# uthree/tinyvc

Measured on AMD Instinct MI355X. Metric: audio-samples/sec (16 kHz) end-to-end VC, higher is better.
Workload: dtype f32 (fp32 in / out / accumulate; channel contractions as two-term fp16 splits on v_mfma_f32_32x32x16_f16: 22-bit significands, three part-products per fp32 product)

## Files before the change

### tinyvc_amd/csrc/api.hip

```cpp
#include <atomic>
#include <cmath>
#include <mutex>

#include <cstdlib>

#include "knn_blob.h"
#include "tvc_common.h"

using namespace tvc;

static std::mutex g_blob_mu;
static std::map<const void*, int64_t> g_blobs;
constexpr size_t kMaxBlobRecords = 4096;
static void blob_record(const void* p, int64_t N) {
    std::lock_guard<std::mutex> lk(g_blob_mu);
    if (g_blobs.size() >= kMaxBlobRecords && !g_blobs.count(p)) g_blobs.clear();
    g_blobs[p] = N;
}
static void blob_forget(const void* p) {
    std::lock_guard<std::mutex> lk(g_blob_mu);
    g_blobs.erase(p);
}
static int blob_check(tvc_ctx* ctx, hipStream_t s, const void* p, int64_t N, const char* what) {
    {
// ... 168 lines not shown
    float* emax = ws.get<float>((size_t)(2 + nslots) * NB);
    float* spec_bound = emax + NB;
    float* enc_slots = spec_bound + NB;
    float* srcmax = c.alpha ? enc_slots + 3 * NB : nullptr;
    float* abound = c.alpha ? ws.get<float>((size_t)NB) : nullptr;
    const int M = ix.M > 0 ? ix.M : 1;
    float* rowmax = ix.per_row ? ws.get<float>((size_t)NB) : nullptr;
    const bool auto_pitch = c.target_f0 != nullptr;
    float* rshift = ix.per_row && c.shifts && !auto_pitch ? ws.get<float>((size_t)NB) : nullptr;
    std::vector<KnnSegIn> segs;
    if (ix.per_row) {
        for (int m = 0; m < M; ++m)
            for (int i = 0; i < NB; ++i) {
                const int r = ctx->rag ? ctx->rag->row[i] : i;
                const int c0 = ctx->rag ? ctx->rag->pre[i] : i * T, nc = ctx->rag ? ctx->rag->tb[i] : T;
                segs.push_back(KnnSegIn{ix.blobs[(size_t)r * M + m], ix.Ns[(size_t)r * M + m], m * B * T + c0, nc});
            }
    } else {
        segs.push_back(KnnSegIn{ix.blob, ix.N, 0, B * T});
    }
    if (ix.per_row && !ws.dry) {
        std::vector<const float*> bl((size_t)NB * M);
        std::vector<int> sh(NB), rows(NB);
        for (int i = 0; i < NB; ++i) {
            const int r = ctx->rag ? ctx->rag->row[i] : i;
            rows[i] = r;
            for (int m = 0; m < M; ++m) bl[(size_t)i * M + m] = ix.blobs[(size_t)r * M + m];
            if (rshift) std::memcpy(&sh[i], &c.shifts[r], sizeof(int));
        }
        if (ix.M > 0) TVC_CHECK(run_knn_blend_bound(ctx, s, bl, rows, M, ix.weights, rowmax));
        else TVC_CHECK(run_knn_amax_rows(ctx, s, bl, rowmax));
        if (rshift) TVC_CHECK(upload_ints(ctx, s, sh, reinterpret_cast<int*>(rshift)));
    }
    size_t m = ws.mark();
    {
        ProfScope ps(ctx, s, ws, "stft");
        TVC_CHECK(run_stft(ctx, s, ws, c.wav, spec, B, L));
    }
    ws.release(m);
    {
        ProfScope ps(ctx, s, ws, "energy");
        TVC_CHECK(run_energy(ctx, s, ws, c.wav, energy, B, L, emax, spec_bound, enc_slots, nslots * NB));
    }
    ws.release(m);
    {
        ProfScope ps(ctx, s, ws, "encoder");
        TVC_CHECK(run_encoder(ctx, s, ws, spec, ssl, f0, nullptr, B, T, spec_bound, enc_slots, auto_pitch ? nullptr : f0s, c.shift, rshift));
        if (c.track && !ws.dry) {
            TVC_CHECK(run_pitch_track(ctx, s, f0, B, T, *c.track, c.target_f0, c.shift, c.shifts, nullptr, nullptr, c.shift_out, f0s));
        } else if (auto_pitch && !ws.dry) {
            std::vector<PitchRow> rows((size_t)NB);
            for (int i = 0; i < NB; ++i) {
                const int r = ctx->rag ? ctx->rag->row[i] : i;
                rows[i] = PitchRow{ctx->rag ? ctx->rag->pre[i] : i * T, ctx->rag ? ctx->rag->tb[i] : T, r, c.shifts ? c.shifts[r] : c.shift};
            }
            TVC_CHECK(run_pitch_match(ctx, s, f0, rows, c.target_f0, nullptr, nullptr, c.shift_out, f0s));
        }
    }
    ws.release(m);
    {
        ProfScope ps(ctx, s, ws, "knn");
        if (ix.M > 0) TVC_CHECK(run_knn_blend(ctx, s, ws, ssl, segs.data(), (int)segs.size(), ix.M, ix.weights, matched, nullptr, B, T, c.alpha));
        else TVC_CHECK(run_knn_segs(ctx, s, ws, ssl, segs.data(), (int)segs.size(), matched, nullptr, B, T, c.alpha));
    }
    ws.release(m);
    const float* idx_bound = ws.dry ? nullptr : (ix.per_row ? rowmax : blob_amax(ix.blob));
    if (c.alpha && !ws.dry) {
        TVC_CHECK(run_ssl_amax(ctx, s, ssl, B, T, srcmax));
        TVC_CHECK(run_knn_alpha_bound(ctx, s, c.alpha, idx_bound, ix.per_row ? 1 : 0, srcmax, abound, NB));
    }
    TVC_CHECK(run_decoder(ctx, s, ws, matched, f0s, energy, c.angle, c.seed, c.wave, nullptr, nullptr, nullptr, B, T, c.alpha && !ws.dry ? abound : idx_bound, emax,
                          c.alpha || ix.per_row ? 1 : 0));
    ws.release(m);
    return 0;
}

static float* const kDryPtr = (float*)(uintptr_t)256;

static int walks_agree(tvc_ctx* ctx, const char* entry, size_t real_peak, size_t measured) {
    return real_peak <= measured ? TVC_OK : fail(ctx, TVC_ERR_WORKSPACE, "%s: the launching walk took %zu workspace bytes, the measuring walk %zu", entry, real_peak, measured);
}

static size_t whole_granules(size_t bytes, size_t granule) { return (bytes + granule - 1) / granule * granule; }
template <class Walk, class Step>
static int run_walks(tvc_ctx* ctx, const char* entry, void* wsp, size_t ws_bytes, size_t granule, Walk&& walk, Step&& before_launch) {
    Ws need(nullptr, 0, true);
    TVC_CHECK(walk(need));
    const size_t bytes = whole_granules(need.peak, granule);
    if (bytes > ws_bytes) return fail(ctx, TVC_ERR_WORKSPACE, "workspace too small: need %zu bytes, got %zu", bytes, ws_bytes);
    TVC_CHECK(before_launch());
    Ws ws(wsp, bytes, false);
    TVC_CHECK(walk(ws));
    return walks_agree(ctx, entry, ws.peak, need.peak);
}
template <class Walk>
static int run_walks(tvc_ctx* ctx, const char* entry, void* wsp, size_t ws_bytes, size_t granule, Walk&& walk) {
    return run_walks(ctx, entry, wsp, ws_bytes, granule, walk, [] { return 0; });
}
template <class Walk>
static int measure(size_t granule, size_t* out_bytes, Walk&& walk) {
    Ws ws(nullptr, 0, true);
    TVC_CHECK(walk(ws));
    *out_bytes = whole_granules(ws.peak, granule) + 4096;
    return TVC_OK;
}
// ... 779 lines not shown
```

### tinyvc_amd/csrc/decoder.hip

```cpp
#include "conv3s.h"
#include "conv_s2.h"
#include "film_s2.h"
#include "gemm_s2.h"
#include "small_kernels.h"
#include "tvc_common.h"

namespace tvc {


__device__ __forceinline__ float div24k(float x) {
    const float r = 1.0f / 24000.0f;
    const float q0 = __fmul_rn(x, r);
    return fmaf(fmaf(-q0, 24000.0f, x), r, q0);
}

__device__ __forceinline__ double wave_incl_scan(double v, int lane) {
#pragma unroll
    for (int o = 1; o < 64; o <<= 1) {
        double u = __shfl_up(v, o);
        if (lane >= o) v += u;
    }
    return v;
}

// ... 104 lines not shown
        }
    }
}

static __global__ __launch_bounds__(256) void noise_ola_kernel(const float* __restrict__ frames, float* __restrict__ source, int B, int T, float* __restrict__ smax, RagDev rg) {
    __shared__ float red[4];
    const long Ls = (long)T * kHop;
    const long b = blockIdx.y;
    long fbase = b * T, sbase = (b * 16 + 15) * Ls;
    if (rg.tb) {
        T = rg.tb[b];
        fbase = rg.pre[b];
        sbase = 15 * Ls + (long)rg.pre[b] * kHop;
    }
    const long L = (long)T * kHop;
    float mx = 0.f;
    for (long i = blockIdx.x * (long)blockDim.x + threadIdx.x; i < L; i += (long)gridDim.x * blockDim.x) {
        int p = (int)i;
        int q = p + kNfft / 2;
        int f_hi = q / kHop;
        if (f_hi > T) f_hi = T;
        int f_lo = (q - (kNfft - 1) + kHop - 1) / kHop;
        if (q - (kNfft - 1) <= 0) f_lo = 0;
        float s = 0.f;
        for (int f = f_lo > 1 ? f_lo : 1; f <= f_hi; ++f)
            s = __fadd_rn(s, frames[(fbase + (f - 1)) * kNfft + (q - f * kHop)]);
        const float v = s / (float)(f_hi - f_lo + 1);
        source[sbase + p] = v;
        mx = fmaxf(mx, fabsf(v));
    }
    amax_flush_wg(smax + b, mx, red);
}

static int run_source_net(tvc_ctx* ctx, hipStream_t s, Ws& ws, const float* content, const float* f0,
                          const float* energy, float* amps, float* kern, int B, int T, const float* cmax, float* xmax_zeroed, hipEvent_t amps_ready = nullptr) {
    const int ncols = B * T;
    float* ef = ws.get<float>((size_t)B * T);
    float* x = ws.get<float>((size_t)B * kSrcCh * T);
    const int NB = ctx->rag ? ctx->rag->B : B;
    float* xmax = xmax_zeroed ? xmax_zeroed : ws.get<float>((size_t)NB);
    if (!ws.dry) {
        hipLaunchKernelGGL(window_max_kernel, dim3(grid_for((long)ncols * 64)), dim3(256), 0, s, energy, ef, (long)B, T, kHop);
        EpiSumCond ep{x, ctx->src_content_in.bias, ef, f0, ctx->src_e_w, ctx->src_e_b, ctx->src_f_w, ctx->src_f_b, kSrcCh, T, ncols};
        int rc = 0;
        if (!gemm_s2_try(&rc, ctx, s, ctx->src_content_in, content, B, kSslDim, T, 0, ep, cmax)) rc = gemm_s_launch<2, 4, 2>(ctx, s, ctx->src_content_in, content, B, kSslDim, T, 0, ep, cmax);
        TVC_CHECK(rc);
    }
    if (!ws.dry && !xmax_zeroed) TVC_HIP(ctx, hipMemsetAsync(xmax, 0, (size_t)NB * sizeof(float), s));
    for (int i = 0; i < 3; ++i) TVC_CHECK(run_convnext(ctx, s, ws, ctx->src_mid[i], x, B, T, i == 2 ? xmax : nullptr));
    if (ws.dry) return 0;
    EpiBias<ACT_ELU1, false> ea{amps, ctx->src_to_amps.bias, nullptr, kHarm, T, ncols, (long)kHarm * T, 0};
    TVC_CHECK((gemm_s_launch<1, 4, 2>(ctx, s, ctx->src_to_amps, x, B, kSrcCh, T, 0, ea, xmax)));
    if (amps_ready) TVC_HIP(ctx, hipEventRecord(amps_ready, s));
    EpiBias<ACT_ELU1, false> ek{kern, ctx->src_to_kernel.bias, nullptr, kBins, T, ncols, (long)kBins * T, 0};
    TVC_CHECK((gemm_s_launch<2, 4, 2>(ctx, s, ctx->src_to_kernel, x, B, kSrcCh, T, 0, ek, xmax)));
    return launch_check(ctx, "source_net");
}

static int run_harm_sums(tvc_ctx* ctx, hipStream_t s, const float* f0, double* csum, int B, int T) {
    const long L = (long)T * kHop;
    const int NB = ctx->rag ? ctx->rag->B : B;
    const int Tg = ctx->rag ? ctx->rag->Tlong : T;
    RagDev rg;
    TVC_CHECK(rag_view(ctx, s, 1, 0, &rg, nullptr));
    const float scale_size = (float)T / (float)L;
    hipLaunchKernelGGL(harm_frame_sum_kernel, dim3((Tg + 3) / 4, NB), dim3(256), 0, s, f0, csum, T, scale_size, rg);
    hipLaunchKernelGGL(harm_frame_scan_kernel, dim3(kHarm, NB), dim3(64), 0, s, csum, T, rg);
    return launch_check(ctx, "harm_sums");
}

int run_dsp(tvc_ctx* ctx, hipStream_t s, Ws& ws, const float* f0, const float* amps, const float* kern, const float* angle, uint64_t seed, float* source, int B, int T,
            float* smax, double* csum, const DspFork* fk) {
    const long L = (long)T * kHop;
    if (!csum) csum = ws.get<double>((size_t)B * kHarm * T);
    float* frames = ws.get<float>((size_t)B * T * kNfft);
// ... 199 lines not shown
                }
            }
            if (C != 48) {
                EpiBias<ACT_NONE, false> ep{xlev[i], u.c5.bias, nullptr, u.cout, lo, nc, (long)u.cout * lo, 0, slot(S_LEV + i), slot(S_UXU + i), u.c5_bw, u.c5_bb, NB};
                if (u.cout == 48) {
                    EpiBiasG8 eg{xlev[i], u.c5.bias, u.cout, lo, nc, slot(S_LEV + i), slot(S_UXU + i), u.c5_bw, u.c5_bb, NB};
                    TVC_CHECK((gemm_s_launch<2, 4, 2>(ctx, s, u.c5, xu, B, C, lo, 0, eg, slot(S_UXU + i))));
                } else if (u.c5.MT6 % 3 == 0) TVC_CHECK((gemm_s_launch<3, 4, 1>(ctx, s, u.c5, xu, B, C, lo, 0, ep, slot(S_UXU + i))));
                else TVC_CHECK((gemm_s_launch<2, 4, 2>(ctx, s, u.c5, xu, B, C, lo, 0, ep, slot(S_UXU + i))));
            }
        }
        ws.release(mk);
        x = xlev[i];
        mx_in = slot(S_LEV + i);
    }
    if (!ws.dry && taps) {
        for (int i = 1; i < 5; ++i)
            if (taps->skips[i] && i == 1)
                hipLaunchKernelGGL(g8_to_planar_kernel, dim3(grid_for((long)B * 48 * len_dn[1])), dim3(256), 0, s, skip[1], taps->skips[1], (long)B, len_dn[1], 48);
            else if (taps->skips[i])
                TVC_HIP(ctx, hipMemcpyAsync(taps->skips[i], skip[i], (size_t)B * ch[4 - i] * len_dn[i] * sizeof(float), hipMemcpyDeviceToDevice, s));
        long l = T;
        for (int i = 0; i < 4; ++i) {
            l *= ctx->ups[i].factor;
            if (taps->ups[i] && ctx->ups[i].cout <= 48)
                hipLaunchKernelGGL(g8_to_planar_kernel, dim3(grid_for((long)B * ctx->ups[i].cout * l)), dim3(256), 0, s, xlev[i], taps->ups[i], (long)B, l, ctx->ups[i].cout);
            else if (taps->ups[i])
                TVC_HIP(ctx, hipMemcpyAsync(taps->ups[i], xlev[i], (size_t)B * ctx->ups[i].cout * l * sizeof(float), hipMemcpyDeviceToDevice, s));
        }
    }
    return ws.dry ? 0 : launch_check(ctx, "filter_net");
}

int run_decoder(tvc_ctx* ctx, hipStream_t s, Ws& ws, const float* content, const float* f0,
                const float* energy, const float* angle, uint64_t seed, float* wave, float* amps_out,
                float* kernel_out, float* source_out, int B, int T, const float* content_bound, const float* energy_bound,
                int content_bound_stride) {
    const long L = (long)T * kHop;
    float* amps = amps_out ? amps_out : ws.get<float>((size_t)B * kHarm * T);
    float* kern = kernel_out ? kernel_out : ws.get<float>((size_t)B * kBins * T);
    float* source = source_out ? source_out : ws.get<float>((size_t)B * 16 * L);
    const int NB = ctx->rag ? ctx->rag->B : B;
    float* cmax = ws.get<float>((size_t)(3 + kFilterSlots) * NB);
    float* smax = cmax + NB;
    float* xmax = smax + NB;
    float* fslots = xmax + NB;
    float* x0 = ws.get<float>((size_t)B * 384 * T);
    double* csum = ws.get<double>((size_t)B * kHarm * T);
    if (!ws.dry) {
        TVC_CHECK(run_slot_prep(ctx, s, cmax, (3 + kFilterSlots) * NB, content_bound ? cmax : nullptr, content_bound, content_bound_stride, 1.f, 0.f, energy_bound ? smax : nullptr,
                                energy_bound, 1, 1.f, 0.f, content_bound ? fslots + (size_t)kFilterSlotX * NB : nullptr, ctx->flt_in_bw, ctx->flt_in_bb,
                                NB));
        if (!content_bound) TVC_CHECK(run_amax_rows(ctx, s, content, B, kSslDim, T, cmax));
        if (!energy_bound) TVC_CHECK(run_amax_rows(ctx, s, energy, B, 1, L, smax));
    }
    SideFork fk(ctx, s);
    if (wave) TVC_CHECK(fk.fork(ws, ctx->ev_fork2, ctx->ev_join2));
    if (fk.forked()) {
        TVC_CHECK(run_harm_sums(ctx, fk.side, f0, csum, B, T));
        ProfScope ps(ctx, fk.side, ws, "filter_net.input@side");
        TVC_CHECK(filter_input_gemm(ctx, fk.side, content, f0, x0, B, T, cmax));
    }
    size_t mk = ws.mark();
    {
        ProfScope ps(ctx, s, ws, "source_net");
        TVC_CHECK(run_source_net(ctx, s, ws, content, f0, energy, amps, kern, B, T, cmax, xmax, fk.forked() ? ctx->ev_amps : nullptr));
    }
    ws.release(mk);
    if (!wave && !source_out) return 0;
    {
        ProfScope ps(ctx, s, ws, "dsp");
        const DspFork df{fk.side, ctx->ev_amps};
        TVC_CHECK(run_dsp(ctx, s, ws, f0, amps, kern, angle, seed, source, B, T, smax, csum, fk.forked() ? &df : nullptr));
        TVC_CHECK(fk.join());
    }
    ws.release(mk);
    if (!wave) return 0;
    ProfScope ps(ctx, s, ws, "filter_net");
    TVC_CHECK(run_filter(ctx, s, ws, content, f0, energy, source, wave, B, T, nullptr, cmax, smax, fslots, content_bound != nullptr, x0, fk.forked()));
    ws.release(mk);
    return 0;
}

}
```

### tinyvc_amd/csrc/encoder.hip

```cpp
#include "conv3s.h"
#include "gemm_s2.h"
#include "cnx_s3.h"
#include "small_kernels.h"
#include "tvc_common.h"

namespace tvc {

constexpr int ENC_MTB = 4, ENC_NWV = 4, ENC_BPC = 2;

template <bool DW, int CPT>
static __global__ __launch_bounds__(1024) void dwconv_ln_kernel(const float* x, float* y,
                                                               const float* __restrict__ dw_w, const float* __restrict__ dw_b,
                                                               const float* __restrict__ g, const float* __restrict__ bta,
                                                               int C, int T, int dil, RagDev rg) {
    constexpr int NW = 16;
    const int rs = T;
    long ubase = (long)blockIdx.y * C * T;
    if (rg.tb) {
        T = rg.tb[blockIdx.y];
        ubase = rg.pre[blockIdx.y];
        if ((int)blockIdx.x * 64 >= T) return;
    }
    __shared__ float red[NW][64];
    constexpr bool STAGE = CPT >= 16;
// ... 321 lines not shown
    for (int j = 0; j < CPW; ++j) {
        const float x = xv[j];
        top.insert(x != x ? INFINITY : x, wave * CPW + j);
    }
#pragma unroll
    for (int e = 0; e < 4; ++e) { sv[wave][e][lane] = top.v[e]; si[wave][e][lane] = top.i[e]; }
    __syncthreads();
    if (wave != 0 || !ok) return;
    for (int w = 1; w < kPdWaves; ++w)
#pragma unroll
        for (int e = 0; e < 4; ++e) top.insert(sv[w][e][lane], si[w][e][lane]);
#pragma unroll
    for (int e = 0; e < 4; ++e) top.i[e] = (unsigned)top.i[e] < (unsigned)kPitchClasses ? top.i[e] : 0;
    const float v0 = top.v[0];
    float e0 = 1.f, e1 = (float)exp((double)(top.v[1] - v0)), e2 = (float)exp((double)(top.v[2] - v0)), e3 = (float)exp((double)(top.v[3] - v0));
    float den = ((e0 + e1) + e2) + e3;
    float acc = __fmul_rn(e0 / den, freq[top.i[0]]);
    acc = __fadd_rn(acc, __fmul_rn(e1 / den, freq[top.i[1]]));
    acc = __fadd_rn(acc, __fmul_rn(e2 / den, freq[top.i[2]]));
    acc = __fadd_rn(acc, __fmul_rn(e3 / den, freq[top.i[3]]));
    const float fv = acc <= 20.f ? 0.f : acc;
    f0[n] = fv;
    if (f0s) f0s[n] = shift_frequency_one(fv, shifts ? shifts[col2b ? col2b[n] : b] : shift);
}

int run_pitch_decode(tvc_ctx* ctx, hipStream_t s, const float* logits, float* f0, int B, int T) {
    if (!ctx->pitch_freq) return fail(ctx, TVC_ERR_STATE, "pitch table not uploaded (tvc_set_pitch_table + tvc_finalize_weights)");
    const long ncols = (long)B * T;
    hipLaunchKernelGGL(pitch_decode_kernel, dim3((unsigned)((ncols + 63) / 64)), dim3(kPdWaves * 64), 0, s, logits, ctx->pitch_freq, f0, B, T, (float*)nullptr, 0.f, (const float*)nullptr, (const int*)nullptr);
    return launch_check(ctx, "pitch_decode");
}

int run_encoder(tvc_ctx* ctx, hipStream_t s, Ws& ws, const float* spec, float* ssl, float* f0,
                float* logits, int B, int T, const float* spec_bound, float* zeroed_slots, float* f0_shifted, float shift, const float* shifts) {
    const int ncols = B * T;
    float* xs = ws.get<float>((size_t)B * kSslCh * T);
    float* xp = ws.get<float>((size_t)B * kPitchCh * T);
    float* lg = logits ? logits : ws.get<float>((size_t)B * kPitchClasses * T);
    const int NB = ctx->rag ? ctx->rag->B : B;
    float* slots = zeroed_slots ? zeroed_slots : ws.get<float>((size_t)3 * NB);
    float *spec_max = slots, *xs_max = slots + NB, *xp_max = slots + 2 * NB;
    if (!ws.dry) {
        if (!zeroed_slots) TVC_HIP(ctx, hipMemsetAsync(slots, 0, (size_t)3 * NB * sizeof(float), s));
        if (spec_bound) spec_max = const_cast<float*>(spec_bound);
        else TVC_CHECK(run_amax_rows(ctx, s, spec, B, kBins, T, spec_max));
        EpiSplit ep{xs, xp, ctx->enc_in.bias, kSslCh, kPitchCh, T, ncols};
        TVC_CHECK((gemm_s_launch_ragged<ENC_MTB, ENC_NWV, ENC_BPC>(ctx, s, ctx->enc_in, spec, B, kBins, T, (long)kBins * T, ep, spec_max)));
        TVC_CHECK(run_layernorm(ctx, s, xs, ctx->ssl_ln_g, ctx->ssl_ln_b, B, kSslCh, T));
        TVC_CHECK(run_layernorm(ctx, s, xp, ctx->pit_ln_g, ctx->pit_ln_b, B, kPitchCh, T));
    }
    const int gtiles = ((ctx->rag ? ctx->rag->Tlong : T) + 63) / 64;
    const size_t ssl_scratch = ((size_t)B * kSslCh * T * 3 + (size_t)NB * kSslCh * 2 * (gtiles + 1)) * sizeof(float) + (size_t)NB * 8 + 4096;
    char* ssl_blk = ws.get<char>(ssl_scratch);
    Ws wssl(ssl_blk, ssl_scratch, ws.dry);
    SideFork fk(ctx, s);
    TVC_CHECK(fk.fork(ws, ctx->ev_fork, ctx->ev_join));
    const hipStream_t sp = fk.side;
    for (int i = 0; i < 4; ++i) TVC_CHECK(run_convnext(ctx, sp, ws, ctx->pit_mid[i], xp, B, T, i == 3 ? xp_max : nullptr));
    if (!ws.dry) {
        EpiBias<ACT_NONE, false> ep{lg, ctx->pit_out.bias, nullptr, kPitchClasses, T, ncols, (long)kPitchClasses * T, 0};
        int rc = 0;
        if (!gemm_s2_try(&rc, ctx, sp, ctx->pit_out, xp, B, kPitchCh, T, 0, ep, xp_max)) rc = gemm_s_launch<ENC_MTB, ENC_NWV, ENC_BPC>(ctx, sp, ctx->pit_out, xp, B, kPitchCh, T, 0, ep, xp_max);
        TVC_CHECK(rc);
        hipLaunchKernelGGL(pitch_decode_kernel, dim3((ncols + 63) / 64), dim3(kPdWaves * 64), 0, sp, lg, ctx->pitch_freq, f0, B, T, f0_shifted, shift, shifts,
                           shifts && ctx->rag ? ctx->rag->d_col2b : (const int*)nullptr);
    }
    TVC_CHECK(fk.end());
    for (int i = 0; i < 6; ++i) TVC_CHECK(run_convnext(ctx, s, wssl, ctx->ssl_mid[i], xs, B, T, i == 5 ? xs_max : nullptr));
    if (wssl.peak > wssl.cap) return fail(ctx, TVC_ERR_WORKSPACE, "encoder: SSL scratch block too small");
    if (ws.dry) return 0;
    {
        EpiBias<ACT_NONE, false> ep{ssl, ctx->ssl_out.bias, nullptr, kSslDim, T, ncols, (long)kSslDim * T, 0};
        int rc = 0;
        if (!gemm_s2_try(&rc, ctx, s, ctx->ssl_out, xs, B, kSslCh, T, 0, ep, xs_max)) rc = gemm_s_launch<ENC_MTB, ENC_NWV, ENC_BPC>(ctx, s, ctx->ssl_out, xs, B, kSslCh, T, 0, ep, xs_max);
        TVC_CHECK(rc);
    }
    TVC_CHECK(fk.join());
    return launch_check(ctx, "encoder");
}

int run_ssl_amax(tvc_ctx* ctx, hipStream_t s, const float* ssl, int B, int T, float* slot) { return run_amax_rows(ctx, s, ssl, B, kSslDim, T, slot); }

}
```

### tinyvc_amd/csrc/frontend.hip

```cpp
#include "small_kernels.h"
#include "tvc_common.h"

namespace tvc {

int run_stft(tvc_ctx* ctx, hipStream_t s, Ws& ws, const float* wav, float* spec, int B, int64_t L) {
    return ws.dry ? 0 : run_stft_fft(ctx, s, wav, spec, B, L);
}

static __global__ void energy_pool_kernel(const float* __restrict__ wav, float* __restrict__ e, int B, int L, int ne) {
    long total = (long)B * ne;
    const int lane = threadIdx.x & 63;
    long wave = (blockIdx.x * (long)blockDim.x + threadIdx.x) >> 6;
    long nwaves = ((long)gridDim.x * blockDim.x) >> 6;
    for (long i = wave; i < total; i += nwaves) {
        int b = (int)(i / ne), j = (int)(i - (long)b * ne);
        const float* x = wav + (long)b * L;
        int lo = 64 * j - 32;
        float m = -INFINITY;
        for (int k = lane; k < 128; k += 64) {
            int p = lo + k;
            if (p >= 0 && p < L) m = fmaxf(m, fabsf(x[p]));
        }
#pragma unroll
        for (int o = 32; o > 0; o >>= 1) m = fmaxf(m, __shfl_xor(m, o));
// ... 62 lines not shown
    const float* p = e + (long)blockIdx.x * ne;
    float m = 0.f;
    for (int j = threadIdx.x; j < ne; j += 256) m = fmaxf(m, p[j]);
#pragma unroll
    for (int o = 32; o > 0; o >>= 1) m = fmaxf(m, __shfl_xor(m, o));
    if ((threadIdx.x & 63) == 0) red[threadIdx.x >> 6] = m;
    __syncthreads();
    if (threadIdx.x == 0) {
        m = fmaxf(fmaxf(red[0], red[1]), fmaxf(red[2], red[3]));
        emax[blockIdx.x] = m;
        if (spec_bound) spec_bound[blockIdx.x] = fmaf(960.5f, m, 0.f);
    }
}

static __global__ __launch_bounds__(256) void pooled_max_rag_kernel(const float* __restrict__ e, RagDev rg, float* __restrict__ emax, float* __restrict__ spec_bound, float* __restrict__ zero, int nz) {
    __shared__ float red[4];
    for (int i = blockIdx.x * 256 + threadIdx.x; i < nz; i += gridDim.x * 256) zero[i] = 0.f;
    const int b = blockIdx.x;
    const int L = rg.tb[b] * kHop, ne = (L + 2 * 32 - 128) / 64 + 1;
    const float* p = e + (15L * rg.pre[b]) / 2;
    float m = 0.f;
    for (int j = threadIdx.x; j < ne; j += 256) m = fmaxf(m, p[j]);
#pragma unroll
    for (int o = 32; o > 0; o >>= 1) m = fmaxf(m, __shfl_xor(m, o));
    if ((threadIdx.x & 63) == 0) red[threadIdx.x >> 6] = m;
    __syncthreads();
    if (threadIdx.x == 0) {
        m = fmaxf(fmaxf(red[0], red[1]), fmaxf(red[2], red[3]));
        emax[b] = m;
        if (spec_bound) spec_bound[b] = fmaf(960.5f, m, 0.f);
    }
}

int run_energy(tvc_ctx* ctx, hipStream_t s, Ws& ws, const float* wav, float* energy, int B, int64_t L, float* emax, float* spec_bound, float* zero, int nz) {
    const int ne = (int)((L + 2 * 32 - 128) / 64 + 1);
    float* e = ws.get<float>((size_t)B * ne + 8);
    if (ws.dry) return 0;
    if (ctx->rag) {
        RagDev rg;
        TVC_CHECK(rag_view(ctx, s, kHop, 0, &rg, nullptr));
        const int gx = ctx->rag->B >= 32 ? 8 : 64;
        hipLaunchKernelGGL(energy_rag_kernel, dim3(gx, ctx->rag->B), dim3(256), 0, s, wav, e, energy, rg, 0);
        if (emax) hipLaunchKernelGGL(pooled_max_rag_kernel, dim3(ctx->rag->B), dim3(256), 0, s, e, rg, emax, spec_bound, zero, nz);
        hipLaunchKernelGGL(energy_rag_kernel, dim3(gx * 4, ctx->rag->B), dim3(256), 0, s, wav, e, energy, rg, 1);
        return launch_check(ctx, "energy (ragged)");
    }
    hipLaunchKernelGGL(energy_pool_kernel, dim3(grid_for((long)B * ne * 64)), dim3(256), 0, s, wav, e, B, (int)L, ne);
    if (emax) hipLaunchKernelGGL(pooled_max_kernel, dim3(B), dim3(256), 0, s, e, ne, emax, spec_bound, zero, nz);
    float scale = (float)ne / (float)L;
    {
        const LerpLaunch ll = lerp_launch((long)B, (int)L);
        hipLaunchKernelGGL(lerp_resize_kernel, ll.grid, dim3(256), 0, s, e, energy, (long)B, ne, (int)L, scale, ll.tx);
    }
    return launch_check(ctx, "energy");
}

static __global__ void shift_kernel(const float* __restrict__ f0, float* __restrict__ out, long n, float shift) {
    for (long i = blockIdx.x * (long)blockDim.x + threadIdx.x; i < n; i += (long)gridDim.x * blockDim.x) out[i] = shift_frequency_one(f0[i], shift);
}

static __global__ __launch_bounds__(256) void uniform_to_angle_kernel(float* __restrict__ u, int64_t n) {
    const int64_t i = 4 * (blockIdx.x * (int64_t)blockDim.x + threadIdx.x);
    const float pi = 3.1415927410125732f;
    if (i + 3 < n && (reinterpret_cast<uintptr_t>(u) & 15) == 0) {
        float4 v = *reinterpret_cast<float4*>(u + i);
        v.x = __fsub_rn(__fmul_rn(__fmul_rn(v.x, 2.f), pi), pi);
        v.y = __fsub_rn(__fmul_rn(__fmul_rn(v.y, 2.f), pi), pi);
        v.z = __fsub_rn(__fmul_rn(__fmul_rn(v.z, 2.f), pi), pi);
        v.w = __fsub_rn(__fmul_rn(__fmul_rn(v.w, 2.f), pi), pi);
        *reinterpret_cast<float4*>(u + i) = v;
    } else {
        for (int64_t k = i; k < n && k < i + 4; ++k) u[k] = __fsub_rn(__fmul_rn(__fmul_rn(u[k], 2.f), pi), pi);
    }
}
int run_uniform_to_angle(tvc_ctx* ctx, hipStream_t s, float* u, int64_t n) {
    const int64_t groups = (n + 3) / 4;
    hipLaunchKernelGGL(uniform_to_angle_kernel, dim3((unsigned)((groups + 255) / 256)), dim3(256), 0, s, u, n);
    return launch_check(ctx, "uniform_to_angle");
}

int run_shift(tvc_ctx* ctx, hipStream_t s, const float* f0, float* out, int64_t n, float semitones) {
    hipLaunchKernelGGL(shift_kernel, dim3(grid_for(n)), dim3(256), 0, s, f0, out, (long)n, semitones);
    return launch_check(ctx, "shift_frequency");
}

constexpr int kPmRows = 256;
struct PitchRowChunk {
// ... 203 lines not shown
```

### tinyvc_amd/csrc/tvc_common.h

```cpp
#pragma once
#include <hip/hip_runtime.h>

#include <atomic>
#include <cstdarg>
#include <cstdint>
#include <cstdio>
#include <cstring>
#include <map>
#include <string>
#include <vector>

#include "../../include/tinyvc_hip.h"
#include "ragged.h"

namespace tvc {

constexpr int kSampleRate = 24000;
constexpr int kNfft = 1920;
constexpr int kHop = 480;
constexpr int kBins = 961;
constexpr int kSslDim = 768;
constexpr int kSslCh = 384;
constexpr int kPitchCh = 128;
constexpr int kPitchClasses = 512;
constexpr int kSrcCh = 128;
constexpr int kHarm = 15;
constexpr int kSolaCross = 1920, kSolaSearch = 1920, kSolaDelay = 3840;
constexpr int kSolaMaxBlock = 1 << 30;
constexpr int kSolaGroups = 8, kSolaPartFloats = 16384;

struct PackedW {
    const float* bias = nullptr;
    const float* A6 = nullptr;
    const float* wscale = nullptr;
    const float* wjoint = nullptr;
    int M = 0, K = 0, Mpad = 0, Kpad = 0, cin = 0, taps = 1, MT6 = 0, S6 = 0;
};

struct ConvNeXtW {
    const float* dw_w = nullptr;
// ... 225 lines not shown
        return e && r == hipSuccess ? hipStreamWaitEvent(s, e, 0) : r;
    }
    int join() { TVC_HIP(ctx, record_and_wait()); return 0; }
    ~SideFork() { (void)record_and_wait(); }
};

inline int launch_check(tvc_ctx* ctx, const char* what) {
    hipError_t e = hipGetLastError();
    if (e != hipSuccess) return fail(ctx, TVC_ERR_HIP, "launch %s: %s", what, hipGetErrorString(e));
    return 0;
}

template <auto... K>
int lds_optin(tvc_ctx* ctx, int bytes, const char* what) {
    static std::atomic<bool> ready_dev[64];
    std::atomic<bool>& ready = ready_dev[ctx->device & 63];
    if (ready.load(std::memory_order_acquire)) return 0;
    for (const void* k : {(const void*)K...}) {
        const hipError_t e = hipFuncSetAttribute(k, hipFuncAttributeMaxDynamicSharedMemorySize, bytes);
        if (e != hipSuccess) return fail(ctx, TVC_ERR_HIP, "%s setup: %s", what, hipGetErrorString(e));
    }
    ready.store(true, std::memory_order_release);
    return 0;
}

void pack_constants(tvc_ctx*, ArenaBuilder*);
void pack_checkpoint(tvc_ctx*, ArenaBuilder*, std::string* missing_enc, std::string* missing_dec);

int run_stft(tvc_ctx*, hipStream_t, Ws&, const float* wav, float* spec, int B, int64_t L);
int run_stft_fft(tvc_ctx*, hipStream_t, const float* wav, float* spec, int B, int64_t L);
int run_noise_ifft(tvc_ctx*, hipStream_t, const float* kern, const float* angle, uint64_t seed, float* frames, int B, int T, bool angle_padded = false);
int run_energy(tvc_ctx*, hipStream_t, Ws&, const float* wav, float* energy, int B, int64_t L, float* emax = nullptr, float* spec_bound = nullptr,
               float* zero = nullptr, int nz = 0);
int run_knn_amax_rows(tvc_ctx*, hipStream_t, const std::vector<const float*>& blobs, float* out);
int run_slot_affine(tvc_ctx*, hipStream_t, float* out, const float* in, int in_stride, float a, float c, int n);
int run_slot_prep(tvc_ctx*, hipStream_t, float* zero, int nz, float* o1, const float* in1, int s1, float a1, float c1, float* o2, const float* in2, int s2, float a2,
                  float c2, float* o3, float a3, float c3, int n);
constexpr int kBlobMagic = 0x54564B4E, kBlobVersion = 2;
constexpr int kFilterSlotX = 2;
constexpr int kFilterSlots = 41;
int run_encoder(tvc_ctx*, hipStream_t, Ws&, const float* spec, float* ssl, float* f0,
                float* logits, int B, int T, const float* spec_bound = nullptr, float* zeroed_slots = nullptr,
                float* f0_shifted = nullptr, float shift = 0.f,
                const float* shifts = nullptr);
int run_pitch_decode(tvc_ctx*, hipStream_t, const float* logits, float* f0, int B, int T);
int run_knn(tvc_ctx*, hipStream_t, Ws&, const float* src, const float* prepared, int64_t N,
            float* out, int64_t* idx_out, int B, int T);
struct KnnSegIn {
    const float* blob;
    int64_t N;
    int col0, ncols;
};
int run_knn_segs(tvc_ctx*, hipStream_t, Ws&, const float* src, const KnnSegIn* in, int nin, float* out, int64_t* idx_out, int B, int T,
                 const float* alpha = nullptr);
int run_knn_blend(tvc_ctx*, hipStream_t, Ws&, const float* src, const KnnSegIn* in, int nin, int M, const float* weights, float* out, int64_t* idx_out,
                  int B, int T, const float* alpha = nullptr);
int run_knn_blend_bound(tvc_ctx*, hipStream_t, const std::vector<const float*>& blobs, const std::vector<int>& rows, int M, const float* weights, float* out);
int run_knn_alpha_bound(tvc_ctx*, hipStream_t, const float* alpha, const float* idx_bound, int stride, const float* srcmax, float* out, int n);
int run_ssl_amax(tvc_ctx*, hipStream_t, const float* ssl, int B, int T, float* slot);

struct ConvertIndex {
    const float* blob = nullptr;
    int64_t N = 0;
    const float* const* blobs = nullptr;
    const int64_t* Ns = nullptr;
    bool per_row = false;
    int M = 0;
    const float* weights = nullptr;
    static ConvertIndex one(const float* blob, int64_t N) { return {blob, N, nullptr, nullptr, false, 0, nullptr}; }
    static ConvertIndex table(const float* const* blobs, const int64_t* Ns) { return {nullptr, 0, blobs, Ns, true, 0, nullptr}; }
    static ConvertIndex blend(const float* const* blobs, const int64_t* Ns, int M, const float* weights) { return {nullptr, 0, blobs, Ns, true, M, weights}; }
};
struct PitchTrackState {
    int start = 0, n = 0, W = 0, min_voiced = 1;
    float slew = 0.f;
    float* ring = nullptr;
    int64_t* count = nullptr;
// ... 2 lines not shown
struct ConvertCall {
    const float* wav = nullptr;
    float* wave = nullptr;
    int B = 0;
    int64_t L = 0;
    const int64_t* lens = nullptr;
    ConvertIndex index;
    float shift = 0.f;
    const float* shifts = nullptr;
    const float* angle = nullptr;
    uint64_t seed = 0;
    const float* target_f0 = nullptr;
    float* shift_out = nullptr;
    const PitchTrackState* track = nullptr;
    const float* alpha = nullptr;
};
int convert_impl(tvc_ctx*, hipStream_t, Ws&, const ConvertCall& c);
int run_knn_topk(tvc_ctx*, hipStream_t, Ws&, const float* src, const float* prepared, int64_t N,
                 float* sims_out, int64_t* idx_out, int B, int T);
int run_knn_general(tvc_ctx*, hipStream_t, Ws&, const float* src, const float* index, int64_t N, int k, int metric, float* out, int64_t* idx_out,
                    float* val_out, int B, int T);
int run_knn_slots(tvc_ctx*, hipStream_t, const float* prepared, int64_t N, const int64_t* idx, float* slots, int64_t nslots);
int run_knn_finish(tvc_ctx*, hipStream_t, const float* slots, float* out, int B, int T);
int run_shift(tvc_ctx*, hipStream_t, const float* f0, float* out, int64_t n, float semitones);
struct PitchRow {
    int start, len, idx;
    float offset;
};
int run_pitch_match(tvc_ctx*, hipStream_t, const float* f0, const std::vector<PitchRow>& rows, const float* target, float* median_out, int* voiced_out,
                    float* shift_out, float* f0s);
int run_pitch_track(tvc_ctx*, hipStream_t, const float* f0, int S, int T, const PitchTrackState& t, const float* target, float offset,
                    const float* offsets, float* median_out, int64_t* count_out, float* shift_out, float* f0s);
int run_uniform_to_angle(tvc_ctx*, hipStream_t, float* u, int64_t n);
int run_decoder(tvc_ctx*, hipStream_t, Ws&, const float* content, const float* f0,
                const float* energy, const float* angle, uint64_t seed, float* wave, float* amps_out,
                float* kernel_out, float* source_out, int B, int T, const float* content_bound = nullptr, const float* energy_bound = nullptr,
                int content_bound_stride = 0);
struct FilterTaps {
    float* skips[5] = {nullptr, nullptr, nullptr, nullptr, nullptr};
    float* ups[4] = {nullptr, nullptr, nullptr, nullptr};
};
int run_filter(tvc_ctx*, hipStream_t, Ws&, const float* content, const float* f0, const float* energy,
               const float* source, float* wave, int B, int T, const FilterTaps* taps = nullptr, const float* cmax = nullptr, const float* smax = nullptr,
               float* zeroed_slots = nullptr, bool x_slot_set = false, float* x_pre = nullptr, bool x_pre_filled = false);
struct DspFork {
    hipStream_t side;
    hipEvent_t amps_ready;
};
int run_dsp(tvc_ctx*, hipStream_t, Ws&, const float* f0, const float* amps, const float* kern, const float* angle, uint64_t seed, float* source, int B, int T,
            float* smax = nullptr, double* csum = nullptr, const DspFork* fk = nullptr);
int sola_geometry(int block, int cross, int search, int delay, int64_t* min_ly, int* latency_min, int* latency_max, char* why, size_t why_bytes);
int run_sola(tvc_ctx*, hipStream_t, const float* y, float* sola_buf, const float* fade_in, float* out, int32_t* shift_out,
             int S, int64_t Ly, int block, int cross, int search, int delay, int use_pv);
int run_stream_push(tvc_ctx* ctx, hipStream_t s, float* buf, const float* blocks, int S, int n, int m);
constexpr int kGateMaxSub = 4096, kGateMaxSubFrame = 1 << 16, kGateMaxCount = 1 << 20;
struct StreamGate {
    int block, sub, look, hold, attack, release;
    float hysteresis_db, range_db;
    const float* threshold_db;
    int32_t* open;
    int32_t* hold_state;
    float* gain;
    float* level_db;
};
int stream_gate_geometry(int block, int sub, int look, int hold, int attack, int release, int* nsub, int* look_samples, char* why, size_t why_bytes);
int run_stream_gate(tvc_ctx*, hipStream_t, const float* x, int64_t n, int64_t base, const int32_t* shift, const float* y, float* out, int S, const StreamGate& g);
int64_t resample_out_len(int64_t n, int orig_freq, int new_freq);
int run_resample(tvc_ctx*, hipStream_t, const float* x, float* y, int rows, int64_t n, int orig_freq, int new_freq);
int stream_resample_geometry(int in_freq, int out_freq, int64_t n_in, int64_t* n_out, int* hist, int* delay);
int stream_resample_prepare(tvc_ctx*, int in_freq, int out_freq);
// ... 34 lines not shown
```

Baseline: 716.4 million.

## Overlap energy resize, window max and decoder slot prep on encoder side stream

Splits the energy stage into a bounds pass, which stays on the main stream, and a resize pass. The resize, the window-max pooling and the decoder slot preparation now run as a tail on the encoder's pitch side stream, so they overlap the SSL ConvNeXt stack. The pitch layernorm also moves onto the side stream by forking earlier. This takes small serial kernels off the critical path, at the cost of keeping more workspace live across stages and adding cross-stream ordering dependencies.

```diff
diff --git a/tinyvc_amd/csrc/api.hip b/tinyvc_amd/csrc/api.hip
--- a/tinyvc_amd/csrc/api.hip
+++ b/tinyvc_amd/csrc/api.hip
@@ -224,20 +224,30 @@
         else TVC_CHECK(run_knn_amax_rows(ctx, s, bl, rowmax));
         if (rshift) TVC_CHECK(upload_ints(ctx, s, sh, reinterpret_cast<int*>(rshift)));
     }
+    float* e = ws.get<float>(energy_pooled_floats(B, L));
+    float* ef = ws.get<float>((size_t)B * T);
+    float* dslots = c.alpha ? nullptr : ws.get<float>((size_t)kDecoderSlots * NB);
+    const float* idx_bound = ws.dry ? nullptr : (ix.per_row ? rowmax : blob_amax(ix.blob));
     size_t m = ws.mark();
     {
         ProfScope ps(ctx, s, ws, "stft");
         TVC_CHECK(run_stft(ctx, s, ws, c.wav, spec, B, L));
     }
     ws.release(m);
-    {
+    if (!ws.dry) {
         ProfScope ps(ctx, s, ws, "energy");
-        TVC_CHECK(run_energy(ctx, s, ws, c.wav, energy, B, L, emax, spec_bound, enc_slots, nslots * NB));
-    }
-    ws.release(m);
+        TVC_CHECK(run_energy_bounds(ctx, s, c.wav, e, B, L, emax, spec_bound, enc_slots, nslots * NB));
+    }
+    const std::function<int(hipStream_t)> decoder_prep = [&](hipStream_t side) {
+        ProfScope ps(ctx, side, ws, "energy.resize+decoder_prep@side");
+        TVC_CHECK(run_energy_resize(ctx, side, c.wav, e, energy, B, L));
+        TVC_CHECK(run_window_max(ctx, side, energy, ef, B, T));
+        if (dslots) TVC_CHECK(run_decoder_slots(ctx, side, dslots, NB, idx_bound, ix.per_row ? 1 : 0, emax));
+        return 0;
+    };
     {
         ProfScope ps(ctx, s, ws, "encoder");
-        TVC_CHECK(run_encoder(ctx, s, ws, spec, ssl, f0, nullptr, B, T, spec_bound, enc_slots, auto_pitch ? nullptr : f0s, c.shift, rshift));
+        TVC_CHECK(run_encoder(ctx, s, ws, spec, ssl, f0, nullptr, B, T, spec_bound, enc_slots, auto_pitch ? nullptr : f0s, c.shift, rshift, &decoder_prep));
         if (c.track && !ws.dry) {
             TVC_CHECK(run_pitch_track(ctx, s, f0, B, T, *c.track, c.target_f0, c.shift, c.shifts, nullptr, nullptr, c.shift_out, f0s));
         } else if (auto_pitch && !ws.dry) {
@@ -256,13 +266,12 @@
         else TVC_CHECK(run_knn_segs(ctx, s, ws, ssl, segs.data(), (int)segs.size(), matched, nullptr, B, T, c.alpha));
     }
     ws.release(m);
-    const float* idx_bound = ws.dry ? nullptr : (ix.per_row ? rowmax : blob_amax(ix.blob));
     if (c.alpha && !ws.dry) {
         TVC_CHECK(run_ssl_amax(ctx, s, ssl, B, T, srcmax));
         TVC_CHECK(run_knn_alpha_bound(ctx, s, c.alpha, idx_bound, ix.per_row ? 1 : 0, srcmax, abound, NB));
     }
     TVC_CHECK(run_decoder(ctx, s, ws, matched, f0s, energy, c.angle, c.seed, c.wave, nullptr, nullptr, nullptr, B, T, c.alpha && !ws.dry ? abound : idx_bound, emax,
-                          c.alpha || ix.per_row ? 1 : 0));
+                          c.alpha || ix.per_row ? 1 : 0, ef, dslots));
     ws.release(m);
     return 0;
 }
diff --git a/tinyvc_amd/csrc/decoder.hip b/tinyvc_amd/csrc/decoder.hip
--- a/tinyvc_amd/csrc/decoder.hip
+++ b/tinyvc_amd/csrc/decoder.hip
@@ -160,15 +160,22 @@
     amax_flush_wg(smax + b, mx, red);
 }
 
+int run_window_max(tvc_ctx* ctx, hipStream_t s, const float* energy, float* ef, int B, int T) {
+    hipLaunchKernelGGL(window_max_kernel, dim3(grid_for((long)B * T * 64)), dim3(256), 0, s, energy, ef, (long)B, T, kHop);
+    return launch_check(ctx, "window_max");
+}
+
 static int run_source_net(tvc_ctx* ctx, hipStream_t s, Ws& ws, const float* content, const float* f0,
-                          const float* energy, float* amps, float* kern, int B, int T, const float* cmax, float* xmax_zeroed, hipEvent_t amps_ready = nullptr) {
+                          const float* energy, float* amps, float* kern, int B, int T, const float* cmax, float* xmax_zeroed, const float* ef_ready = nullptr,
+                          hipEvent_t amps_ready = nullptr) {
     const int ncols = B * T;
-    float* ef = ws.get<float>((size_t)B * T);
+    float* ef_own = ef_ready ? nullptr : ws.get<float>((size_t)B * T);
     float* x = ws.get<float>((size_t)B * kSrcCh * T);
     const int NB = ctx->rag ? ctx->rag->B : B;
     float* xmax = xmax_zeroed ? xmax_zeroed : ws.get<float>((size_t)NB);
     if (!ws.dry) {
-        hipLaunchKernelGGL(window_max_kernel, dim3(grid_for((long)ncols * 64)), dim3(256), 0, s, energy, ef, (long)B, T, kHop);
+        if (!ef_ready) TVC_CHECK(run_window_max(ctx, s, energy, ef_own, B, T));
+        const float* ef = ef_ready ? ef_ready : ef_own;
         EpiSumCond ep{x, ctx->src_content_in.bias, ef, f0, ctx->src_e_w, ctx->src_e_b, ctx->src_f_w, ctx->src_f_b, kSrcCh, T, ncols};
         int rc = 0;
         if (!gemm_s2_try(&rc, ctx, s, ctx->src_content_in, content, B, kSslDim, T, 0, ep, cmax)) rc = gemm_s_launch<2, 4, 2>(ctx, s, ctx->src_content_in, content, B, kSslDim, T, 0, ep, cmax);
@@ -434,25 +441,29 @@
     return ws.dry ? 0 : launch_check(ctx, "filter_net");
 }
 
+int run_decoder_slots(tvc_ctx* ctx, hipStream_t s, float* slots, int nb, const float* content_bound, int content_bound_stride, const float* energy_bound) {
+    float *cmax = slots, *smax = slots + nb, *fslots = slots + (size_t)3 * nb;
+    return run_slot_prep(ctx, s, slots, kDecoderSlots * nb, content_bound ? cmax : nullptr, content_bound, content_bound_stride, 1.f, 0.f, energy_bound ? smax : nullptr, energy_bound,
+                         1, 1.f, 0.f, content_bound ? fslots + (size_t)kFilterSlotX * nb : nullptr, ctx->flt_in_bw, ctx->flt_in_bb, nb);
+}
+
 int run_decoder(tvc_ctx* ctx, hipStream_t s, Ws& ws, const float* content, const float* f0,
                 const float* energy, const float* angle, uint64_t seed, float* wave, float* amps_out,
                 float* kernel_out, float* source_out, int B, int T, const float* content_bound, const float* energy_bound,
-                int content_bound_stride) {
+                int content_bound_stride, const float* ef, float* slots_ready) {
     const long L = (long)T * kHop;
     float* amps = amps_out ? amps_out : ws.get<float>((size_t)B * kHarm * T);
     float* kern = kernel_out ? kernel_out : ws.get<float>((size_t)B * kBins * T);
     float* source = source_out ? source_out : ws.get<float>((size_t)B * 16 * L);
     const int NB = ctx->rag ? ctx->rag->B : B;
-    float* cmax = ws.get<float>((size_t)(3 + kFilterSlots) * NB);
+    float* cmax = slots_ready ? slots_ready : ws.get<float>((size_t)kDecoderSlots * NB);
     float* smax = cmax + NB;
     float* xmax = smax + NB;
     float* fslots = xmax + NB;
     float* x0 = ws.get<float>((size_t)B * 384 * T);
     double* csum = ws.get<double>((size_t)B * kHarm * T);
     if (!ws.dry) {
-        TVC_CHECK(run_slot_prep(ctx, s, cmax, (3 + kFilterSlots) * NB, content_bound ? cmax : nullptr, content_bound, content_bound_stride, 1.f, 0.f, energy_bound ? smax : nullptr,
-                                energy_bound, 1, 1.f, 0.f, content_bound ? fslots + (size_t)kFilterSlotX * NB : nullptr, ctx->flt_in_bw, ctx->flt_in_bb,
-                                NB));
+        if (!slots_ready) TVC_CHECK(run_decoder_slots(ctx, s, cmax, NB, content_bound, content_bound_stride, energy_bound));
         if (!content_bound) TVC_CHECK(run_amax_rows(ctx, s, content, B, kSslDim, T, cmax));
         if (!energy_bound) TVC_CHECK(run_amax_rows(ctx, s, energy, B, 1, L, smax));
     }
@@ -466,7 +477,7 @@
     size_t mk = ws.mark();
     {
         ProfScope ps(ctx, s, ws, "source_net");
-        TVC_CHECK(run_source_net(ctx, s, ws, content, f0, energy, amps, kern, B, T, cmax, xmax, fk.forked() ? ctx->ev_amps : nullptr));
+        TVC_CHECK(run_source_net(ctx, s, ws, content, f0, energy, amps, kern, B, T, cmax, xmax, ef, fk.forked() ? ctx->ev_amps : nullptr));
     }
     ws.release(mk);
     if (!wave && !source_out) return 0;
diff --git a/tinyvc_amd/csrc/encoder.hip b/tinyvc_amd/csrc/encoder.hip
--- a/tinyvc_amd/csrc/encoder.hip
+++ b/tinyvc_amd/csrc/encoder.hip
@@ -377,7 +377,8 @@
 }
 
 int run_encoder(tvc_ctx* ctx, hipStream_t s, Ws& ws, const float* spec, float* ssl, float* f0,
-                float* logits, int B, int T, const float* spec_bound, float* zeroed_slots, float* f0_shifted, float shift, const float* shifts) {
+                float* logits, int B, int T, const float* spec_bound, float* zeroed_slots, float* f0_shifted, float shift, const float* shifts,
+                const std::function<int(hipStream_t)>* side_tail) {
     const int ncols = B * T;
     float* xs = ws.get<float>((size_t)B * kSslCh * T);
     float* xp = ws.get<float>((size_t)B * kPitchCh * T);
@@ -385,6 +386,7 @@
     const int NB = ctx->rag ? ctx->rag->B : B;
     float* slots = zeroed_slots ? zeroed_slots : ws.get<float>((size_t)3 * NB);
     float *spec_max = slots, *xs_max = slots + NB, *xp_max = slots + 2 * NB;
+    SideFork fk(ctx, s);
     if (!ws.dry) {
         if (!zeroed_slots) TVC_HIP(ctx, hipMemsetAsync(slots, 0, (size_t)3 * NB * sizeof(float), s));
         if (spec_bound) spec_max = const_cast<float*>(spec_bound);
@@ -392,14 +394,13 @@
         EpiSplit ep{xs, xp, ctx->enc_in.bias, kSslCh, kPitchCh, T, ncols};
         TVC_CHECK((gemm_s_launch_ragged<ENC_MTB, ENC_NWV, ENC_BPC>(ctx, s, ctx->enc_in, spec, B, kBins, T, (long)kBins * T, ep, spec_max)));
         TVC_CHECK(run_layernorm(ctx, s, xs, ctx->ssl_ln_g, ctx->ssl_ln_b, B, kSslCh, T));
-        TVC_CHECK(run_layernorm(ctx, s, xp, ctx->pit_ln_g, ctx->pit_ln_b, B, kPitchCh, T));
+        TVC_CHECK(fk.fork(ws, ctx->ev_fork, ctx->ev_join));
+        TVC_CHECK(run_layernorm(ctx, fk.side, xp, ctx->pit_ln_g, ctx->pit_ln_b, B, kPitchCh, T));
     }
     const int gtiles = ((ctx->rag ? ctx->rag->Tlong : T) + 63) / 64;
     const size_t ssl_scratch = ((size_t)B * kSslCh * T * 3 + (size_t)NB * kSslCh * 2 * (gtiles + 1)) * sizeof(float) + (size_t)NB * 8 + 4096;
     char* ssl_blk = ws.get<char>(ssl_scratch);
     Ws wssl(ssl_blk, ssl_scratch, ws.dry);
-    SideFork fk(ctx, s);
-    TVC_CHECK(fk.fork(ws, ctx->ev_fork, ctx->ev_join));
     const hipStream_t sp = fk.side;
     for (int i = 0; i < 4; ++i) TVC_CHECK(run_convnext(ctx, sp, ws, ctx->pit_mid[i], xp, B, T, i == 3 ? xp_max : nullptr));
     if (!ws.dry) {
@@ -409,6 +410,7 @@
         TVC_CHECK(rc);
         hipLaunchKernelGGL(pitch_decode_kernel, dim3((ncols + 63) / 64), dim3(kPdWaves * 64), 0, sp, lg, ctx->pitch_freq, f0, B, T, f0_shifted, shift, shifts,
                            shifts && ctx->rag ? ctx->rag->d_col2b : (const int*)nullptr);
+        if (side_tail) TVC_CHECK((*side_tail)(sp));
     }
     TVC_CHECK(fk.end());
     for (int i = 0; i < 6; ++i) TVC_CHECK(run_convnext(ctx, s, wssl, ctx->ssl_mid[i], xs, B, T, i == 5 ? xs_max : nullptr));
diff --git a/tinyvc_amd/csrc/frontend.hip b/tinyvc_amd/csrc/frontend.hip
--- a/tinyvc_amd/csrc/frontend.hip
+++ b/tinyvc_amd/csrc/frontend.hip
@@ -118,27 +118,43 @@
     }
 }
 
-int run_energy(tvc_ctx* ctx, hipStream_t s, Ws& ws, const float* wav, float* energy, int B, int64_t L, float* emax, float* spec_bound, float* zero, int nz) {
+size_t energy_pooled_floats(int B, int64_t L) { return (size_t)B * (size_t)((L + 2 * 32 - 128) / 64 + 1) + 8; }
+
+int run_energy_bounds(tvc_ctx* ctx, hipStream_t s, const float* wav, float* e, int B, int64_t L, float* emax, float* spec_bound, float* zero, int nz) {
     const int ne = (int)((L + 2 * 32 - 128) / 64 + 1);
-    float* e = ws.get<float>((size_t)B * ne + 8);
-    if (ws.dry) return 0;
     if (ctx->rag) {
         RagDev rg;
         TVC_CHECK(rag_view(ctx, s, kHop, 0, &rg, nullptr));
         const int gx = ctx->rag->B >= 32 ? 8 : 64;
-        hipLaunchKernelGGL(energy_rag_kernel, dim3(gx, ctx->rag->B), dim3(256), 0, s, wav, e, energy, rg, 0);
+        hipLaunchKernelGGL(energy_rag_kernel, dim3(gx, ctx->rag->B), dim3(256), 0, s, wav, e, (float*)nullptr, rg, 0);
         if (emax) hipLaunchKernelGGL(pooled_max_rag_kernel, dim3(ctx->rag->B), dim3(256), 0, s, e, rg, emax, spec_bound, zero, nz);
-        hipLaunchKernelGGL(energy_rag_kernel, dim3(gx * 4, ctx->rag->B), dim3(256), 0, s, wav, e, energy, rg, 1);
-        return launch_check(ctx, "energy (ragged)");
+        return launch_check(ctx, "energy bounds (ragged)");
     }
     hipLaunchKernelGGL(energy_pool_kernel, dim3(grid_for((long)B * ne * 64)), dim3(256), 0, s, wav, e, B, (int)L, ne);
     if (emax) hipLaunchKernelGGL(pooled_max_kernel, dim3(B), dim3(256), 0, s, e, ne, emax, spec_bound, zero, nz);
+    return launch_check(ctx, "energy bounds");
+}
+
+int run_energy_resize(tvc_ctx* ctx, hipStream_t s, const float* wav, const float* e, float* energy, int B, int64_t L) {
+    if (ctx->rag) {
+        RagDev rg;
+        TVC_CHECK(rag_view(ctx, s, kHop, 0, &rg, nullptr));
+        const int gx = ctx->rag->B >= 32 ? 8 : 64;
+        hipLaunchKernelGGL(energy_rag_kernel, dim3(gx * 4, ctx->rag->B), dim3(256), 0, s, wav, const_cast<float*>(e), energy, rg, 1);
+        return launch_check(ctx, "energy resize (ragged)");
+    }
+    const int ne = (int)((L + 2 * 32 - 128) / 64 + 1);
     float scale = (float)ne / (float)L;
-    {
-        const LerpLaunch ll = lerp_launch((long)B, (int)L);
-        hipLaunchKernelGGL(lerp_resize_kernel, ll.grid, dim3(256), 0, s, e, energy, (long)B, ne, (int)L, scale, ll.tx);
-    }
-    return launch_check(ctx, "energy");
+    const LerpLaunch ll = lerp_launch((long)B, (int)L);
+    hipLaunchKernelGGL(lerp_resize_kernel, ll.grid, dim3(256), 0, s, e, energy, (long)B, ne, (int)L, scale, ll.tx);
+    return launch_check(ctx, "energy resize");
+}
+
+int run_energy(tvc_ctx* ctx, hipStream_t s, Ws& ws, const float* wav, float* energy, int B, int64_t L, float* emax, float* spec_bound, float* zero, int nz) {
+    float* e = ws.get<float>(energy_pooled_floats(B, L));
+    if (ws.dry) return 0;
+    TVC_CHECK(run_energy_bounds(ctx, s, wav, e, B, L, emax, spec_bound, zero, nz));
+    return run_energy_resize(ctx, s, wav, e, energy, B, L);
 }
 
 static __global__ void shift_kernel(const float* __restrict__ f0, float* __restrict__ out, long n, float shift) {
diff --git a/tinyvc_amd/csrc/tvc_common.h b/tinyvc_amd/csrc/tvc_common.h
--- a/tinyvc_amd/csrc/tvc_common.h
+++ b/tinyvc_amd/csrc/tvc_common.h
@@ -6,6 +6,7 @@
 #include <cstdint>
 #include <cstdio>
 #include <cstring>
+#include <functional>
 #include <map>
 #include <string>
 #include <vector>
@@ -297,6 +298,9 @@
 int run_noise_ifft(tvc_ctx*, hipStream_t, const float* kern, const float* angle, uint64_t seed, float* frames, int B, int T, bool angle_padded = false);
 int run_energy(tvc_ctx*, hipStream_t, Ws&, const float* wav, float* energy, int B, int64_t L, float* emax = nullptr, float* spec_bound = nullptr,
                float* zero = nullptr, int nz = 0);
+size_t energy_pooled_floats(int B, int64_t L);
+int run_energy_bounds(tvc_ctx*, hipStream_t, const float* wav, float* e, int B, int64_t L, float* emax, float* spec_bound, float* zero, int nz);
+int run_energy_resize(tvc_ctx*, hipStream_t, const float* wav, const float* e, float* energy, int B, int64_t L);
 int run_knn_amax_rows(tvc_ctx*, hipStream_t, const std::vector<const float*>& blobs, float* out);
 int run_slot_affine(tvc_ctx*, hipStream_t, float* out, const float* in, int in_stride, float a, float c, int n);
 int run_slot_prep(tvc_ctx*, hipStream_t, float* zero, int nz, float* o1, const float* in1, int s1, float a1, float c1, float* o2, const float* in2, int s2, float a2,
@@ -307,7 +311,8 @@
 int run_encoder(tvc_ctx*, hipStream_t, Ws&, const float* spec, float* ssl, float* f0,
                 float* logits, int B, int T, const float* spec_bound = nullptr, float* zeroed_slots = nullptr,
                 float* f0_shifted = nullptr, float shift = 0.f,
-                const float* shifts = nullptr);
+                const float* shifts = nullptr,
+                const std::function<int(hipStream_t)>* side_tail = nullptr);
 int run_pitch_decode(tvc_ctx*, hipStream_t, const float* logits, float* f0, int B, int T);
 int run_knn(tvc_ctx*, hipStream_t, Ws&, const float* src, const float* prepared, int64_t N,
             float* out, int64_t* idx_out, int B, int T);
@@ -376,10 +381,13 @@
 int run_pitch_track(tvc_ctx*, hipStream_t, const float* f0, int S, int T, const PitchTrackState& t, const float* target, float offset,
                     const float* offsets, float* median_out, int64_t* count_out, float* shift_out, float* f0s);
 int run_uniform_to_angle(tvc_ctx*, hipStream_t, float* u, int64_t n);
+constexpr int kDecoderSlots = 3 + kFilterSlots;
 int run_decoder(tvc_ctx*, hipStream_t, Ws&, const float* content, const float* f0,
                 const float* energy, const float* angle, uint64_t seed, float* wave, float* amps_out,
                 float* kernel_out, float* source_out, int B, int T, const float* content_bound = nullptr, const float* energy_bound = nullptr,
-                int content_bound_stride = 0);
+                int content_bound_stride = 0, const float* ef = nullptr, float* slots_ready = nullptr);
+int run_window_max(tvc_ctx*, hipStream_t, const float* energy, float* ef, int B, int T);
+int run_decoder_slots(tvc_ctx*, hipStream_t, float* slots, int nb, const float* content_bound, int content_bound_stride, const float* energy_bound);
 struct FilterTaps {
     float* skips[5] = {nullptr, nullptr, nullptr, nullptr, nullptr};
     float* ups[4] = {nullptr, nullptr, nullptr, nullptr};
```

New measurement: 719.2 million (median of 4 runs). About the same (+0.4%).
